# jonasrothfuss/ProMP

Measured on NVIDIA H100. Metric: env_steps_per_sec, higher is better.
Workload: dtype f32

## Files before the change

### promp_b200/csrc/policy_tc.cuh

```cuda
#pragma once
#include "mlp_tile.cuh"

namespace promp {

constexpr int TBT = 128;
constexpr int TC_HID = 64;
constexpr int SCA = TBT * 16 + 16;
constexpr int SCW = TC_HID * 16 + 16;
constexpr int TILE_A_BYTES = 16 * SCA;
constexpr int TILE_W_BYTES = 16 * SCW;

__device__ __forceinline__ int core_off(int r, int c, int sc) {
    return (c >> 2) * sc + (r >> 3) * 128 + (r & 7) * 16 + ((c & 3) << 2);
}
__device__ __forceinline__ float tf32_trunc(float x) { return __uint_as_float(__float_as_uint(x) & 0xffffe000u); }

template <int DO, int DA>
struct SmallLayout {
    static constexpr int W0 = 0;
    static constexpr int B0 = W0 + DO * TC_HID;
    static constexpr int B1 = B0 + TC_HID;
    static constexpr int W2 = B1 + TC_HID;
    static constexpr int B2 = W2 + TC_HID * DA;
    static constexpr int LS = B2 + DA;
    static constexpr int SIZE = (LS + DA + 3) / 4 * 4;
};

template <int DO, int DA, int NQ>
struct GradTcSmem {
    static constexpr int DOP = DOPad<DO>::V;
    alignas(16) unsigned char W1T_hi[TILE_W_BYTES];
    alignas(16) unsigned char W1T_lo[TILE_W_BYTES];
    alignas(16) unsigned char W1_hi[TILE_W_BYTES];
    alignas(16) unsigned char W1_lo[TILE_W_BYTES];
    alignas(16) unsigned char A0[TILE_A_BYTES];
    alignas(16) unsigned char A1[TILE_A_BYTES];
    alignas(16) unsigned char LO[TILE_A_BYTES];
    alignas(16) float Ps[SmallLayout<DO, DA>::SIZE];
    alignas(16) float X[TBT * DOP];
    float MUP[NQ * TBT * DA];
    float DMU[TBT * DA];
    float red[3 * 4 * NQ];
    HeadIn<DA> hin;
    HeadOld<DA> hold;
    int last;
};


__device__ __forceinline__ void mma_tf32_16n8k8(float (&c)[4], const uint32_t (&a)[4], const uint32_t (&b)[2]) {
    asm volatile("mma.sync.aligned.m16n8k8.row.col.f32.tf32.tf32.f32 {%0,%1,%2,%3}, {%4,%5,%6,%7}, {%8,%9}, {%0,%1,%2,%3};\n"
                 : "+f"(c[0]), "+f"(c[1]), "+f"(c[2]), "+f"(c[3])
                 : "r"(a[0]), "r"(a[1]), "r"(a[2]), "r"(a[3]), "r"(b[0]), "r"(b[1]));
}
__device__ __forceinline__ void split_tf32(float x, uint32_t& hi, uint32_t& lo) {
    hi = __float_as_uint(x) & 0xffffe000u;
    lo = __float_as_uint(x - __uint_as_float(hi));
}
template <bool COLSUM, int NT, bool UNIT = false>
__device__ __forceinline__ void wgrad_mma_tile(const unsigned char* __restrict__ At, const unsigned char* __restrict__ Dt,
                                               float scale, int warp, int lane, float (&acc)[NT][4], float (&csum)[NT]) {
    const int g = lane >> 2, t = lane & 3;
    const int k0 = 16 * (warp & 3) + g, j0 = 8 * NT * (warp >> 2) + g;
    const unsigned char* ap = At + (k0 >> 2) * SCA + (k0 & 3) * 4 + t * 32;
    const unsigned char* dp = Dt + (j0 >> 2) * SCA + (j0 & 3) * 4 + t * 32;
#pragma unroll 2
    for (int s = 0; s < TBT / 8; ++s) {
        uint32_t ah[4], al[4], bh[NT][2], bl[NT][2];
        split_tf32(*reinterpret_cast<const float*>(ap + s * 128), ah[0], al[0]);
        split_tf32(*reinterpret_cast<const float*>(ap + s * 128 + 2 * SCA), ah[1], al[1]);
        split_tf32(*reinterpret_cast<const float*>(ap + s * 128 + 16), ah[2], al[2]);
        split_tf32(*reinterpret_cast<const float*>(ap + s * 128 + 2 * SCA + 16), ah[3], al[3]);
#pragma unroll
        for (int nt = 0; nt < NT; ++nt) {
            const float d0 = *reinterpret_cast<const float*>(dp + nt * 2 * SCA + s * 128);
            const float d1 = *reinterpret_cast<const float*>(dp + nt * 2 * SCA + s * 128 + 16);
            if (COLSUM) csum[nt] += d0 + d1;
            split_tf32(UNIT ? d0 : scale * d0, bh[nt][0], bl[nt][0]);
            split_tf32(UNIT ? d1 : scale * d1, bh[nt][1], bl[nt][1]);
        }
#pragma unroll
        for (int nt = 0; nt < NT; ++nt) mma_tf32_16n8k8(acc[nt], al, bh[nt]);
#pragma unroll
        for (int nt = 0; nt < NT; ++nt) mma_tf32_16n8k8(acc[nt], ah, bl[nt]);
#pragma unroll
        for (int nt = 0; nt < NT; ++nt) mma_tf32_16n8k8(acc[nt], ah, bh[nt]);
    }
}
template <int NT>
__device__ __forceinline__ int wgrad_mma_index(int warp, int lane, int nt, int i) {
    const int g = lane >> 2, t = lane & 3;
    return (16 * (warp & 3) + g + 8 * (i >> 1)) * TC_HID + 8 * NT * (warp >> 2) + 8 * nt + 2 * t + (i & 1);
}

__device__ __forceinline__ uint64_t wg_desc(const unsigned char* p) {
    const uint32_t a = static_cast<uint32_t>(__cvta_generic_to_shared(p));
    return (uint64_t)((a & 0x3ffff) >> 4) | ((uint64_t)(SCW >> 4) << 16) | ((uint64_t)(128 >> 4) << 32);
}
__device__ __forceinline__ void wg_fence() { asm volatile("wgmma.fence.sync.aligned;\n" ::: "memory"); }
__device__ __forceinline__ void wg_commit() { asm volatile("wgmma.commit_group.sync.aligned;\n" ::: "memory"); }
__device__ __forceinline__ void wg_wait() { asm volatile("wgmma.wait_group.sync.aligned 0;\n" ::: "memory"); }
constexpr int WG_DEPTH = 0;
__device__ __forceinline__ void wg_wait_depth() { asm volatile("wgmma.wait_group.sync.aligned %0;\n" ::"n"(WG_DEPTH) : "memory"); }
__device__ __forceinline__ void wg_fence_weights() { asm volatile("fence.proxy.async.shared::cta;\n" ::: "memory"); }
template <int LNT>
__device__ __forceinline__ void wg_pin(float (&acc)[LNT][4]) {
#pragma unroll
    for (int nt = 0; nt < LNT; ++nt)
#pragma unroll
        for (int i = 0; i < 4; ++i) asm volatile("" : "+f"(acc[nt][i])::"memory");
}

template <int LNT>
__device__ __forceinline__ void wgmma_tf32(float (&d)[LNT][4], const uint32_t (&a)[4], uint64_t desc);
template <>
__device__ __forceinline__ void wgmma_tf32<4>(float (&d)[4][4], const uint32_t (&a)[4], uint64_t desc) {
    asm volatile(
        "wgmma.mma_async.sync.aligned.m64n32k8.f32.tf32.tf32 "
        "{%0,%1,%2,%3,%4,%5,%6,%7,%8,%9,%10,%11,%12,%13,%14,%15}, {%16,%17,%18,%19}, %20, 1, 1, 1;\n"
        : "+f"(d[0][0]), "+f"(d[0][1]), "+f"(d[0][2]), "+f"(d[0][3]), "+f"(d[1][0]), "+f"(d[1][1]), "+f"(d[1][2]), "+f"(d[1][3]),
          "+f"(d[2][0]), "+f"(d[2][1]), "+f"(d[2][2]), "+f"(d[2][3]), "+f"(d[3][0]), "+f"(d[3][1]), "+f"(d[3][2]), "+f"(d[3][3])
        : "r"(a[0]), "r"(a[1]), "r"(a[2]), "r"(a[3]), "l"(desc));
}
template <>
__device__ __forceinline__ void wgmma_tf32<8>(float (&d)[8][4], const uint32_t (&a)[4], uint64_t desc) {
    asm volatile(
        "wgmma.mma_async.sync.aligned.m64n64k8.f32.tf32.tf32 "
        "{%0,%1,%2,%3,%4,%5,%6,%7,%8,%9,%10,%11,%12,%13,%14,%15,"
        "%16,%17,%18,%19,%20,%21,%22,%23,%24,%25,%26,%27,%28,%29,%30,%31}, {%32,%33,%34,%35}, %36, 1, 1, 1;\n"
        : "+f"(d[0][0]), "+f"(d[0][1]), "+f"(d[0][2]), "+f"(d[0][3]), "+f"(d[1][0]), "+f"(d[1][1]), "+f"(d[1][2]), "+f"(d[1][3]),
          "+f"(d[2][0]), "+f"(d[2][1]), "+f"(d[2][2]), "+f"(d[2][3]), "+f"(d[3][0]), "+f"(d[3][1]), "+f"(d[3][2]), "+f"(d[3][3]),
          "+f"(d[4][0]), "+f"(d[4][1]), "+f"(d[4][2]), "+f"(d[4][3]), "+f"(d[5][0]), "+f"(d[5][1]), "+f"(d[5][2]), "+f"(d[5][3]),
          "+f"(d[6][0]), "+f"(d[6][1]), "+f"(d[6][2]), "+f"(d[6][3]), "+f"(d[7][0]), "+f"(d[7][1]), "+f"(d[7][2]), "+f"(d[7][3])
        : "r"(a[0]), "r"(a[1]), "r"(a[2]), "r"(a[3]), "l"(desc));
}
template <int LNT>
__device__ __forceinline__ void layer_gemm_issue(float (&acc)[LNT][4], const unsigned char* __restrict__ a,
                                                 const unsigned char* __restrict__ b_hi, const unsigned char* __restrict__ b_lo,
                                                 int warp, int lane) {
    const int g = lane >> 2, t = lane & 3;
    const unsigned char* ap = a + (warp & 7) * 256 + g * 16 + t * 4;
    const int bo = (warp >> 3) * LNT * 128;
#pragma unroll 1
    for (int s = 0; s < TC_HID / 8; ++s) {
        const uint64_t dh = wg_desc(b_hi + bo + 2 * s * SCW), dl = wg_desc(b_lo + bo + 2 * s * SCW);
        uint32_t ah[4], al[4];
        const unsigned char* as = ap + 2 * s * SCA;
        split_tf32(*reinterpret_cast<const float*>(as), ah[0], al[0]);
        split_tf32(*reinterpret_cast<const float*>(as + 128), ah[1], al[1]);
        split_tf32(*reinterpret_cast<const float*>(as + SCA), ah[2], al[2]);
        split_tf32(*reinterpret_cast<const float*>(as + SCA + 128), ah[3], al[3]);
        wg_fence();
        wgmma_tf32<LNT>(acc, al, dh);
        wgmma_tf32<LNT>(acc, ah, dl);
        wgmma_tf32<LNT>(acc, ah, dh);
        wg_commit();
        wg_wait_depth();
    }
}
template <int LNT>
__device__ __forceinline__ void zero_frag(float (&acc)[LNT][4]) {
#pragma unroll
    for (int nt = 0; nt < LNT; ++nt) acc[nt][0] = acc[nt][1] = acc[nt][2] = acc[nt][3] = 0.f;
}
template <int LNT>
__device__ __forceinline__ int frag_off(int warp, int lane, int nt, int h) {
    return core_off(16 * (warp & 7) + (lane >> 2) + 8 * h, 8 * (LNT * (warp >> 3) + nt) + 2 * (lane & 3), SCA);
}
template <int LNT>
__device__ __forceinline__ void store_frag(const float (&acc)[LNT][4], unsigned char* tile, int warp, int lane) {
#pragma unroll
    for (int nt = 0; nt < LNT; ++nt)
#pragma unroll
        for (int h = 0; h < 2; ++h)
            *reinterpret_cast<float2*>(tile + frag_off<LNT>(warp, lane, nt, h)) = make_float2(acc[nt][2 * h], acc[nt][2 * h + 1]);
}
template <int CW>
__device__ __forceinline__ void load_row(const unsigned char* tile, int r, int c0, float (&v)[CW]) {
#pragma unroll
    for (int c4 = 0; c4 < CW / 4; ++c4) {
        const float4 x = *reinterpret_cast<const float4*>(tile + core_off(r, c0 + 4 * c4, SCA));
        v[4 * c4] = x.x, v[4 * c4 + 1] = x.y, v[4 * c4 + 2] = x.z, v[4 * c4 + 3] = x.w;
    }
}

#ifdef PROMP_EXP_CLOCKS
__device__ unsigned long long g_chain_clk[16];
__device__ long long g_chain_last[1024];
#define CCLK(i)                                                                                  \
    do {                                                                                         \
        if (threadIdx.x == 0) {                                                                  \
            const long long t_ = clock64();                                                      \
            atomicAdd(&g_chain_clk[i], (unsigned long long)(t_ - g_chain_last[blockIdx.x]));     \
            g_chain_last[blockIdx.x] = t_;                                                       \
        }                                                                                        \
    } while (0)
#define CCNT(i)                                            \
    do {                                                   \
        if (threadIdx.x == 0) atomicAdd(&g_chain_clk[i], 1ull); \
    } while (0)
#else
#define CCLK(i)
#define CCNT(i)
#endif
struct ItemSched {
    int ntiles, g_lo, g_hi;
    int item, first_item, n_items;
    const int* ready_prev;
    int* ready_mine;
    __device__ __forceinline__ int my_slot(int) const { return item; }
    __device__ __forceinline__ int n_contrib(int) const { return n_items; }
    __device__ __forceinline__ int contrib_slot(int, int i) const { return first_item + i; }
    __device__ __forceinline__ void clk(int i) const { CCLK(i); }
    __device__ __forceinline__ void wait_task(int m) const {
        if (ready_prev == nullptr) return;
        if (threadIdx.x == 0) {
            int v;
            unsigned spins = 0;
            long long t0 = 0;
            do {
                asm volatile("ld.acquire.gpu.global.s32 %0, [%1];\n" : "=r"(v) : "l"(ready_prev + m) : "memory");
                if (v == 0 && (++spins & 0xfffu) == 0) {
                    const long long t = clock64();
                    if (t0 == 0) t0 = t;
                    else if (t - t0 > 8000000000ll) {
                        __trap();
                    }
                }
            } while (v == 0);
        }
        __syncthreads();
        CCLK(1);
    }
    __device__ __forceinline__ void publish_task(int m) const {
        __threadfence();
        __syncthreads();
        if (threadIdx.x == 0) asm volatile("st.release.gpu.global.s32 [%0], %1;\n" ::"l"(ready_mine + m), "r"(1) : "memory");
        CCNT(7);
    }
    static __device__ __forceinline__ float ldp(const float* p) { return __ldcg(p); }
    static __device__ __forceinline__ float4 ldp4(const float4* p) { return __ldcg(p); }
};

#ifdef PROMP_EXP_CLOCKS
__device__ unsigned long long g_phase_clk[16];
#define PCLK(i)                                                   \
    do {                                                          \
        if (blockIdx.x == 0 && threadIdx.x == 0) {                \
            const long long t_ = clock64();                       \
            s_clk[i] += (unsigned long long)(t_ - s_last);        \
            s_last = t_;                                          \
        }                                                         \
    } while (0)
#else
#define PCLK(i)
#endif
template <int DO, int DA, int NQ, class Act, class Sched, int ADV = ADV_SAMPLE>
__device__ __forceinline__ void grad_tc_tiles(const PolicyArgs& A, GradTcSmem<DO, DA, NQ>& S, const Sched& sc,
                                              const float*& cached_th) {
    constexpr int HID = TC_HID;
    using L = PLayout<DO, DA, HID>;
    using SL = SmallLayout<DO, DA>;
    using SM = GradTcSmem<DO, DA, NQ>;
    constexpr int TCT = 128 * NQ, CW = TC_HID / NQ, NW = TCT / 32, NT = 8 / NQ;
    constexpr int LNT = 64 / NW;
    constexpr int DOP = SM::DOP;
    constexpr int PSTRIDE = L::P + PSTAT;
    constexpr int NPART = TCT / HID, BPP = TBT / NPART;

#ifdef PROMP_EXP_CLOCKS
    __shared__ unsigned long long s_clk[16];
    __shared__ long long s_last;
    if (threadIdx.x == 0) {
        for (int i = 0; i < 16; ++i) s_clk[i] = 0;
        s_last = clock64();
    }
#endif

    const int tid = threadIdx.x, lane = tid & 31, warp = tid >> 5;
    const int qd = warp & 3, cq = warp >> 2;
    const int r = qd * 32 + lane, c0 = CW * cq;
    const int cj = tid & (HID - 1), cp = tid / HID;
    const int dO = obs_dim_of<DO, DA>(A), dA = act_dim_of<DO, DA>(A);
    const int N = A.N;
    const float kl_eff = kl_coeff_eff(A);
    float invN = 1.0f / (float)N;
    int Nm = N;
    const bool want_grad = A.grad != nullptr;
    const float* th = nullptr;
    HeadIn<DA>& hin = S.hin;

    float gW1[NT][4], gB1f[NT], gW0p[DO], gW2p[DA], gB0c, gB2w[DA], gLSw[DA];
    float s_obj, s_kl, s_ratio;
    auto zero_acc = [&]() {
#pragma unroll
        for (int a = 0; a < NT; ++a) gW1[a][0] = gW1[a][1] = gW1[a][2] = gW1[a][3] = gB1f[a] = 0.f;
#pragma unroll
        for (int i = 0; i < DO; ++i) gW0p[i] = 0.f;
#pragma unroll
        for (int d = 0; d < DA; ++d) gW2p[d] = 0.f;
#pragma unroll
        for (int d = 0; d < DA; ++d) gB2w[d] = gLSw[d] = 0.f;
        gB0c = 0.f;
        s_obj = s_kl = s_ratio = 0.f;
    };
    auto load_task = [&](int m) {
        sc.wait_task(m);
        if (A.n_valid) { Nm = __ldg(A.n_valid + m); invN = 1.0f / (float)max(Nm, 1); }
        th = A.params + (int64_t)m * A.param_stride;
        const bool reload = th != cached_th;
        cached_th = th;
        if (reload) __syncthreads();
        for (int i = tid; reload && i < DO * HID + HID; i += TCT) S.Ps[SL::W0 + i] = Sched::ldp(th + L::W0 + i);
        for (int i = tid; reload && i < HID; i += TCT) S.Ps[SL::B1 + i] = Sched::ldp(th + L::B1 + i);
        for (int i = tid; reload && i < HID * DA + 2 * DA; i += TCT) S.Ps[SL::W2 + i] = Sched::ldp(th + L::W2 + i);
        for (int u = tid; reload && u < HID * HID / 4; u += TCT) {
            float4 w, wl;
            {
                const int jg = u % (HID / 4), k = u / (HID / 4);
                w = Sched::ldp4(reinterpret_cast<const float4*>(th + L::W1 + k * HID + 4 * jg));
                wl = make_float4(w.x - tf32_trunc(w.x), w.y - tf32_trunc(w.y), w.z - tf32_trunc(w.z), w.w - tf32_trunc(w.w));
                const int off = jg * SCW + (k >> 3) * 128 + (k & 7) * 16;
                *reinterpret_cast<float4*>(S.W1_hi + off) = make_float4(tf32_trunc(w.x), tf32_trunc(w.y), tf32_trunc(w.z), tf32_trunc(w.w));
                *reinterpret_cast<float4*>(S.W1_lo + off) = wl;
            }
            {
                const int j = u % HID, kg = u / HID;
                const float* src = th + L::W1 + 4 * kg * HID + j;
// ... 154 lines not shown
                    mu[d] = sm;
                }
                float a[DA], mo[DA], lso[DA], adv;
                if constexpr (XPRE) {
#pragma unroll
                    for (int d = 0; d < DA; ++d) a[d] = ha[d], mo[d] = hmo[d], lso[d] = hlso[d];
                    adv = hadv;
                } else {
                    adv = load_head_sample<DA, ADV>(A, g0 + r, m, dA, A.ls_per_sample, a, mo, lso);
                }
                HeadOut<DA> o;
                out_forward<Act, DA>(mu);
                if (A.ls_per_sample) {
                    HeadOld<DA> ho;
                    head_old_from<DA>(lso, ho, dA);
                    gaussian_head<DA>(hin, ho, mu, a, mo, adv, A.obj_kind, A.clip_eps, o, dA);
                } else {
                    gaussian_head<DA>(hin, S.hold, mu, a, mo, adv, A.obj_kind, A.clip_eps, o, dA);
                }
                grad_signal<DA>(hin, o, A.obj_scale, kl_eff, invN, dmu, dls);
                out_grad_back<Act, DA>(mu, dmu);
                s_obj += o.obj;
                s_kl += o.kl;
                s_ratio += o.ratio;
            } else {
#pragma unroll
                for (int d = 0; d < DA; ++d) dmu[d] = dls[d] = 0.f;
            }
#pragma unroll
            for (int d = 0; d < DA; ++d) {
                S.DMU[r * DA + d] = dmu[d];
                gB2w[d] += dmu[d], gLSw[d] += dls[d];
            }
        }
        if (!want_grad) continue;
        __syncthreads();
        PCLK(4);
        {
            const int b0 = cp * BPP;
            const unsigned char* colp = S.A1 + core_off(b0, cj, SCA);
            const float* dmu0 = S.DMU + b0 * DA;
#pragma unroll(BPP <= 16 ? 2 : 1)
            for (int b8 = 0; b8 < BPP; b8 += 8)
#pragma unroll
            for (int b1 = 0; b1 < 8; ++b1) {
                const int bb = b8 + b1;
                const float h = *reinterpret_cast<const float*>(colp + (bb >> 3) * 128 + (bb & 7) * 16);
#pragma unroll
                for (int d = 0; d < DA; ++d) gW2p[d] = fmaf(h, dmu0[bb * DA + d], gW2p[d]);
            }
        }
        __syncthreads();
        PCLK(5);
        {
            float dm[DA];
#pragma unroll
            for (int d = 0; d < DA; ++d) dm[d] = S.DMU[r * DA + d];
#pragma unroll
            for (int c4 = 0; c4 < CW / 4; ++c4) {
                float v[4];
#pragma unroll
                for (int e = 0; e < 4; ++e) {
                    const int c = 4 * c4 + e;
                    float dh = 0.f;
#pragma unroll
                    for (int d = 0; d < DA; ++d) dh = fmaf(dm[d], S.Ps[SL::W2 + (c0 + c) * DA + d], dh);
                    v[e] = dh * Act::d(h2[c]);
                }
                *reinterpret_cast<float4*>(S.A1 + core_off(r, c0 + 4 * c4, SCA)) = make_float4(v[0], v[1], v[2], v[3]);
            }
        }
        __syncthreads();
        PCLK(6);
        wgrad_mma_tile<true, NT, true>(S.A0, S.A1, 1.f, warp, lane, gW1, gB1f);
        PCLK(7);
        {
            float acc[LNT][4];
            zero_frag<LNT>(acc);
            layer_gemm_issue<LNT>(acc, S.A1, S.W1_hi, S.W1_lo, warp, lane);
            wg_wait();
            wg_pin<LNT>(acc);
            __syncthreads();
            PCLK(8);
#pragma unroll
            for (int nt = 0; nt < LNT; ++nt)
#pragma unroll
                for (int h = 0; h < 2; ++h) {
                    float2* p = reinterpret_cast<float2*>(S.A0 + frag_off<LNT>(warp, lane, nt, h));
                    const float2 hv = *p;
                    *p = make_float2(acc[nt][2 * h] * Act::d(hv.x), acc[nt][2 * h + 1] * Act::d(hv.y));
                }
        }
        __syncthreads();
        PCLK(9);
        {
            const int b0 = cp * BPP;
            const unsigned char* colp = S.A0 + core_off(b0, cj, SCA);
            const float* x0 = S.X + b0 * DOP;
#pragma unroll(BPP <= 16 ? 2 : 1)
            for (int b8 = 0; b8 < BPP; b8 += 8)
#pragma unroll
            for (int b1 = 0; b1 < 8; ++b1) {
                const int bb = b8 + b1;
                const float d1 = *reinterpret_cast<const float*>(colp + (bb >> 3) * 128 + (bb & 7) * 16);
                gB0c += d1;
#pragma unroll
                for (int i = 0; i < DO; ++i) gW0p[i] = fmaf(x0[bb * DOP + i], d1, gW0p[i]);
            }
        }
    }
    PCLK(10);
    if (cur_m >= 0) flush(cur_m);
    PCLK(11);
#ifdef PROMP_EXP_CLOCKS
    if (blockIdx.x == 0 && threadIdx.x == 0)
        for (int i = 0; i < 16; ++i) g_phase_clk[i] += s_clk[i];
#endif
}

template <int DO, int DA, int NQ, class Act, int ADV = ADV_SAMPLE>
__device__ __forceinline__ void policy_grad_tc_body(const PolicyArgs& A) {
    using SM = GradTcSmem<DO, DA, NQ>;
    using L = PLayout<DO, DA, TC_HID>;
    extern __shared__ __align__(16) unsigned char smem_raw[];
    SM& S = *reinterpret_cast<SM*>(smem_raw);
    if (reuse_hit<L::P>(A.skip_flag, A.params, A.skip_theta)) return;
    reuse_produce<L::P, L::LS, DA>(A);
    const UniformSched sc(A.M, A.N, A.q, A.kmax, TBT);
    const float* cached_th = nullptr;
    grad_tc_tiles<DO, DA, NQ, Act, UniformSched, ADV>(A, S, sc, cached_th);
}
template <int DO, int DA, int NQ>
__global__ void __launch_bounds__(128 * NQ, 1) policy_grad_tc_kernel(PolicyArgs A) { policy_grad_tc_body<DO, DA, NQ, ActTanh>(A); }
template <int DO, int DA, int NQ>
__global__ void __launch_bounds__(128 * NQ, 1) policy_grad_tc_relu_kernel(PolicyArgs A) { policy_grad_tc_body<DO, DA, NQ, ActRelu>(A); }
template <int DO, int DA, int NQ>
__global__ void __launch_bounds__(128 * NQ, 1) policy_grad_tc_explore_kernel(PolicyArgs A) {
    policy_grad_tc_body<DO, DA, NQ, ActTanh, ADV_TASK>(A);
}
template <int DO, int DA, int NQ>
__global__ void __launch_bounds__(128 * NQ, 1) policy_grad_tc_explore_relu_kernel(PolicyArgs A) {
    policy_grad_tc_body<DO, DA, NQ, ActRelu, ADV_TASK>(A);
}
template <int DO, int DA, int NQ, class Hid>
__global__ void __launch_bounds__(128 * NQ, 1) policy_grad_tc_otanh_kernel(PolicyArgs A) {
    policy_grad_tc_body<DO, DA, NQ, OutTanh<Hid>>(A);
}
template <int DO, int DA, int NQ, class Hid>
__global__ void __launch_bounds__(128 * NQ, 1) policy_grad_tc_explore_otanh_kernel(PolicyArgs A) {
    policy_grad_tc_body<DO, DA, NQ, OutTanh<Hid>, ADV_TASK>(A);
}


template <int DO, int DA, int NQ>
struct HvpTcSmem {
    static constexpr int DOP = DOPad<DO>::V;
    alignas(16) unsigned char WB[4][TILE_W_BYTES];
    alignas(16) unsigned char H1[TILE_A_BYTES];
    alignas(16) unsigned char R1[TILE_A_BYTES];
    alignas(16) unsigned char T2a[TILE_A_BYTES];
    alignas(16) unsigned char T2b[TILE_A_BYTES];
    alignas(16) float Ps[SmallLayout<DO, DA>::SIZE];
    alignas(16) float Vs[SmallLayout<DO, DA>::SIZE];
    float DMU[TBT * DA];
    float CMU[TBT * DA];
    float red[3 * 4 * NQ];
    HeadIn<DA> hin;
    HeadOld<DA> hold;
    int last;
};

template <int DO, int DA, int NQ, class Act, class Sched>
__device__ __forceinline__ void hvp_tc_tiles(const PolicyArgs& A, HvpTcSmem<DO, DA, NQ>& S, const Sched& sc,
                                             const float*& cached_th) {
    constexpr int HID = TC_HID;
    using L = PLayout<DO, DA, HID>;
    using SL = SmallLayout<DO, DA>;
    using SM = HvpTcSmem<DO, DA, NQ>;
    constexpr int TCT = 128 * NQ, CW = TC_HID / NQ, NW = TCT / 32, NT = 8 / NQ;
    constexpr int LNT = 64 / NW;
    constexpr int DOP = SM::DOP;
    constexpr int PSTRIDE = L::P + PSTAT;
    constexpr int NPART = TCT / HID, BPP = TBT / NPART;

    float* const sX = reinterpret_cast<float*>(S.T2a);
    float* const sMUP = reinterpret_cast<float*>(S.WB[0]);
    static_assert(TBT * DOP * 4 <= TILE_A_BYTES && NQ * TBT * 2 * DA * 4 <= 2 * TILE_W_BYTES, "aliased buffers must fit");

    const int tid = threadIdx.x, lane = tid & 31, warp = tid >> 5;
    const int qd = warp & 3, cq = warp >> 2;
    const int r = qd * 32 + lane, c0 = CW * cq;
    const int cj = tid & (HID - 1), cp = tid / HID;
    const int dO = obs_dim_of<DO, DA>(A), dA = act_dim_of<DO, DA>(A);
    const int N = A.N;
    const float kl_eff = kl_coeff_eff(A);
    float invN = 1.0f / (float)N;
    int Nm = N;
    const float ac = -A.inner_lr;
    const float* th = nullptr;
    const float* vg = nullptr;
    HeadIn<DA>& hin = S.hin;
    float rls[DA];

    float gW1[NT][4], gB1f[NT], gW0p[DO], gW2p[DA], gB0c, gB2w[DA], gLSw[DA];
    float s_obj, s_kl, s_ratio;
    auto zero_acc = [&]() {
#pragma unroll
        for (int a = 0; a < NT; ++a) gW1[a][0] = gW1[a][1] = gW1[a][2] = gW1[a][3] = gB1f[a] = 0.f;
#pragma unroll
        for (int i = 0; i < DO; ++i) gW0p[i] = 0.f;
#pragma unroll
        for (int d = 0; d < DA; ++d) gW2p[d] = 0.f;
#pragma unroll
        for (int d = 0; d < DA; ++d) gB2w[d] = gLSw[d] = 0.f;
        gB0c = 0.f;
        s_obj = s_kl = s_ratio = 0.f;
    };
    const bool vec_ro = A.out != A.vec;
    const float* const al = A.step_size;
    auto ldv = [&](const float* p) {
        const float v = vec_ro ? Sched::ldp(p) : __ldcg(p);
        return al ? __ldg(al + (p - vg)) * v : v;
    };
    auto ldv4 = [&](const float4* p) {
        const float4 v = vec_ro ? Sched::ldp4(p) : __ldcg(p);
        if (!al) return v;
        const float4 a = __ldg(reinterpret_cast<const float4*>(al + (reinterpret_cast<const float*>(p) - vg)));
        return make_float4(a.x * v.x, a.y * v.y, a.z * v.z, a.w * v.w);
    };
    auto load_task = [&](int m) {
        sc.wait_task(m);
        if (A.n_valid) { Nm = __ldg(A.n_valid + m); invN = 1.0f / (float)max(Nm, 1); }
        th = A.params + (int64_t)m * A.param_stride;
        vg = A.vec + (int64_t)m * L::P;
        __syncthreads();
        const bool reload_p = th != cached_th;
        cached_th = th;
        for (int i = tid; i < DO * HID + HID; i += TCT) {
            if (reload_p) S.Ps[SL::W0 + i] = Sched::ldp(th + L::W0 + i);
            S.Vs[SL::W0 + i] = ldv(vg + L::W0 + i);
        }
        for (int i = tid; i < HID; i += TCT) {
            if (reload_p) S.Ps[SL::B1 + i] = Sched::ldp(th + L::B1 + i);
            S.Vs[SL::B1 + i] = ldv(vg + L::B1 + i);
        }
        for (int i = tid; i < HID * DA + 2 * DA; i += TCT) {
            if (reload_p) S.Ps[SL::W2 + i] = Sched::ldp(th + L::W2 + i);
            S.Vs[SL::W2 + i] = ldv(vg + L::W2 + i);
        }
        __syncthreads();
        if (tid == 0) head_setup<DA>(A, S.Ps + SL::LS, m, dA, hin, &S.hold);
        __syncthreads();
#pragma unroll
        for (int d = 0; d < DA; ++d) rls[d] = S.Vs[SL::LS + d] * hin.ls_mask[d];
    };
    auto load_weights = [&](bool fwd) {
        for (int u = tid; u < HID * HID / 4; u += TCT) {
            float4 w, v;
            int off;
            if (fwd) {
                const int j = u % HID, kg = u / HID;
                const float* sw = th + L::W1 + 4 * kg * HID + j;
                const float* sv = vg + L::W1 + 4 * kg * HID + j;
                w = make_float4(Sched::ldp(sw), Sched::ldp(sw + HID), Sched::ldp(sw + 2 * HID), Sched::ldp(sw + 3 * HID));
                v = make_float4(ldv(sv), ldv(sv + HID), ldv(sv + 2 * HID), ldv(sv + 3 * HID));
                off = kg * SCW + (j >> 3) * 128 + (j & 7) * 16;
            } else {
                const int jg = u % (HID / 4), k = u / (HID / 4);
                w = Sched::ldp4(reinterpret_cast<const float4*>(th + L::W1 + k * HID + 4 * jg));
                v = ldv4(reinterpret_cast<const float4*>(vg + L::W1 + k * HID + 4 * jg));
                v = make_float4(ac * v.x, ac * v.y, ac * v.z, ac * v.w);
                off = jg * SCW + (k >> 3) * 128 + (k & 7) * 16;
            }
            *reinterpret_cast<float4*>(S.WB[0] + off) = make_float4(tf32_trunc(w.x), tf32_trunc(w.y), tf32_trunc(w.z), tf32_trunc(w.w));
            *reinterpret_cast<float4*>(S.WB[1] + off) =
                make_float4(w.x - tf32_trunc(w.x), w.y - tf32_trunc(w.y), w.z - tf32_trunc(w.z), w.w - tf32_trunc(w.w));
            *reinterpret_cast<float4*>(S.WB[2] + off) = make_float4(tf32_trunc(v.x), tf32_trunc(v.y), tf32_trunc(v.z), tf32_trunc(v.w));
            *reinterpret_cast<float4*>(S.WB[3] + off) =
                make_float4(v.x - tf32_trunc(v.x), v.y - tf32_trunc(v.y), v.z - tf32_trunc(v.z), v.w - tf32_trunc(v.w));
        }
        wg_fence_weights();
    };
    auto flush = [&](int m) {
        sc.clk(3);
        float* part = A.partial + (int64_t)sc.my_slot(m) * PSTRIDE;
        float* scr = reinterpret_cast<float*>(S.T2a);
        __syncthreads();
#pragma unroll
        for (int nt = 0; nt < NT; ++nt)
#pragma unroll
            for (int i = 0; i < 4; ++i) part[L::W1 + wgrad_mma_index<NT>(warp, lane, nt, i)] = gW1[nt][i];
#pragma unroll
        for (int nt = 0; nt < NT; ++nt) {
            float c = gB1f[nt];
            c += __shfl_xor_sync(0xffffffffu, c, 1);
            c += __shfl_xor_sync(0xffffffffu, c, 2);
            if ((lane & 3) == 0 && (warp & 3) == 0) part[L::B1 + 8 * NT * (warp >> 2) + 8 * nt + (lane >> 2)] = c;
        }
        scr[cp * HID + cj] = gB0c;
        __syncthreads();
        if (tid < HID) {
            float s = 0.f;
            for (int p = 0; p < NPART; ++p) s += scr[p * HID + tid];
            part[L::B0 + tid] = s;
        }
        __syncthreads();
#pragma unroll
        for (int d = 0; d < DA; ++d) {
            const float s1 = warp_sum(gB2w[d]), s2 = warp_sum(gLSw[d]);
            if (cq == 0 && lane == 0) scr[qd * 2 * DA + d] = s1, scr[qd * 2 * DA + DA + d] = s2;
        }
        __syncthreads();
        if (tid < 2 * DA) part[L::B2 + tid] = scr[tid] + scr[2 * DA + tid] + scr[4 * DA + tid] + scr[6 * DA + tid];
        __syncthreads();
        flush_tail<TCT, 8, 2 * TILE_A_BYTES / 4, DO, DA, HID>(A, sc, m, invN, true, part, scr, S.red, S.last, gW0p, gW2p, s_obj, s_kl, s_ratio,
                                        HvpEpilogue<L::P>{A, vg, m});
    };

    constexpr int XR = (TBT * DOP) / TCT;
    constexpr bool XPRE = (TBT * DOP) % TCT == 0 && XR >= 1 && XR <= 2 && DA <= 2;
    float xq[XPRE ? XR : 1], xc[XPRE ? XR : 1], ha[DA], hmo[DA], hlso[DA], hadv = 0.f;
    auto fetch_x = [&](int g_, float (&dst)[XPRE ? XR : 1]) {
        const int m_ = g_ / sc.ntiles, n0_ = (g_ - m_ * sc.ntiles) * TBT;
        const int nb_ = max(0, min(TBT, (A.n_valid ? __ldg(A.n_valid + m_) : N) - n0_));
#pragma unroll
        for (int e = 0; e < (XPRE ? XR : 1); ++e) {
            const int i = tid + e * TCT, b = i / DOP, c = i % DOP;
            dst[e] = (b < nb_ && c < dO) ? __ldg(A.obs + ((int64_t)m_ * N + n0_ + b) * dO + c) : 0.f;
        }
    };
    int cur_m = -1;
    for (int g = sc.g_lo; g < sc.g_hi; ++g) {
        const int m = g / sc.ntiles, tile = g - m * sc.ntiles;
        if (m != cur_m) {
            if (cur_m >= 0) flush(cur_m);
            load_task(m);
            sc.clk(2);
            zero_acc();
            cur_m = m;
        }
        const int n0 = tile * TBT, nb = max(0, min(TBT, Nm - n0));
        const int64_t g0 = (int64_t)m * N + n0;
        __syncthreads();
        auto load_x = [&]() {
            for (int i = tid; i < TBT * DOP; i += TCT) {
                const int b = i / DOP, c = i % DOP;
                sX[i] = (b < nb && c < dO) ? __ldg(A.obs + (g0 + b) * dO + c) : 0.f;
            }
        };
        if constexpr (XPRE) {
            if (g == sc.g_lo) fetch_x(g, xq);
#pragma unroll
            for (int e = 0; e < XR; ++e) xc[e] = xq[e], sX[tid + e * TCT] = xc[e];
            if (g + 1 < sc.g_hi) fetch_x(g + 1, xq);
            if (cq == 0 && r < nb) hadv = load_head_sample<DA>(A, g0 + r, m, dA, A.ls_per_sample, ha, hmo, hlso);
        } else {
            load_x();
        }
        load_weights(true);
        __syncthreads();
        {
            float x[DO];
#pragma unroll
            for (int i = 0; i < DO; ++i) x[i] = sX[r * DOP + i];
#pragma unroll
            for (int c4 = 0; c4 < CW / 4; ++c4) {
                float h[4], r1[4];
#pragma unroll
                for (int e = 0; e < 4; ++e) {
                    const int c = c0 + 4 * c4 + e;
                    float z = S.Ps[SL::B0 + c], rz = S.Vs[SL::B0 + c];
#pragma unroll
                    for (int i = 0; i < DO; ++i) {
                        z = fmaf(x[i], S.Ps[SL::W0 + i * HID + c], z);
                        rz = fmaf(x[i], S.Vs[SL::W0 + i * HID + c], rz);
                    }
                    h[e] = Act::f(z);
                    r1[e] = Act::d(h[e]) * rz;
                }
                const int off = core_off(r, c0 + 4 * c4, SCA);
                *reinterpret_cast<float4*>(S.H1 + off) = make_float4(h[0], h[1], h[2], h[3]);
                *reinterpret_cast<float4*>(S.R1 + off) = make_float4(r1[0], r1[1], r1[2], r1[3]);
            }
        }
        __syncthreads();
        {
            float acc[LNT][4];
            zero_frag<LNT>(acc);
            layer_gemm_issue<LNT>(acc, S.H1, S.WB[0], S.WB[1], warp, lane);
            wg_wait();
            wg_pin<LNT>(acc);
            store_frag<LNT>(acc, S.T2a, warp, lane);
            zero_frag<LNT>(acc);
            layer_gemm_issue<LNT>(acc, S.R1, S.WB[0], S.WB[1], warp, lane);
            layer_gemm_issue<LNT>(acc, S.H1, S.WB[2], S.WB[3], warp, lane);
            wg_wait();
            wg_pin<LNT>(acc);
            store_frag<LNT>(acc, S.T2b, warp, lane);
        }
        __syncthreads();
        float h2[CW], r2[CW];
        load_row<CW>(S.T2a, r, c0, h2);
        load_row<CW>(S.T2b, r, c0, r2);
        {
            float mup[DA], rmup[DA];
#pragma unroll
            for (int d = 0; d < DA; ++d) mup[d] = rmup[d] = 0.f;
#pragma unroll
            for (int c4 = 0; c4 < CW / 4; ++c4) {
#pragma unroll
                for (int e = 0; e < 4; ++e) {
                    const int c = 4 * c4 + e;
                    h2[c] = Act::f(h2[c] + S.Ps[SL::B1 + c0 + c]);
                    r2[c] = Act::d(h2[c]) * (r2[c] + S.Vs[SL::B1 + c0 + c]);
#pragma unroll
                    for (int d = 0; d < DA; ++d) {
                        const float w2 = S.Ps[SL::W2 + (c0 + c) * DA + d];
                        mup[d] = fmaf(h2[c], w2, mup[d]);
                        rmup[d] = fmaf(r2[c], w2, fmaf(h2[c], S.Vs[SL::W2 + (c0 + c) * DA + d], rmup[d]));
                    }
                }
                const int off = core_off(r, c0 + 4 * c4, SCA);
                *reinterpret_cast<float4*>(S.T2a + off) = make_float4(h2[4 * c4], h2[4 * c4 + 1], h2[4 * c4 + 2], h2[4 * c4 + 3]);
                *reinterpret_cast<float4*>(S.T2b + off) = make_float4(r2[4 * c4], r2[4 * c4 + 1], r2[4 * c4 + 2], r2[4 * c4 + 3]);
            }
#pragma unroll
            for (int d = 0; d < DA; ++d) {
                sMUP[((cq * TBT + r) * 2 + 0) * DA + d] = mup[d];
                sMUP[((cq * TBT + r) * 2 + 1) * DA + d] = rmup[d];
            }
        }
        __syncthreads();
        if (cq == 0) {
            float dmu[DA], cmu[DA], cls[DA];
            if (r < nb) {
                float mu[DA], rmu[DA];
#pragma unroll
                for (int d = 0; d < DA; ++d) {
                    float sm = S.Ps[SL::B2 + d], sr = S.Vs[SL::B2 + d];
#pragma unroll
                    for (int q = 0; q < NQ; ++q) sm += sMUP[((q * TBT + r) * 2 + 0) * DA + d], sr += sMUP[((q * TBT + r) * 2 + 1) * DA + d];
                    mu[d] = sm;
                    rmu[d] = sr;
                }
                float a[DA], mo[DA], lso[DA], adv;
                if constexpr (XPRE) {
#pragma unroll
                    for (int d = 0; d < DA; ++d) a[d] = ha[d], mo[d] = hmo[d], lso[d] = hlso[d];
                    adv = hadv;
                } else {
                    adv = load_head_sample<DA>(A, g0 + r, m, dA, A.ls_per_sample, a, mo, lso);
                }
                HeadOut<DA> o;
                out_forward_tangent<Act, DA>(mu, rmu);
                if (A.ls_per_sample) {
                    HeadOld<DA> ho;
                    head_old_from<DA>(lso, ho, dA);
                    gaussian_head<DA>(hin, ho, mu, a, mo, adv, A.obj_kind, A.clip_eps, o, dA);
                } else {
                    gaussian_head<DA>(hin, S.hold, mu, a, mo, adv, A.obj_kind, A.clip_eps, o, dA);
                }
                hvp_signal<DA>(hin, o, rmu, rls, A.obj_kind, kl_eff, invN, ac, dA, dmu, cmu, cls);
                out_hvp_back<Act, DA>(mu, rmu, ac, dmu, cmu);
                s_obj += o.obj;
                s_kl += o.kl;
                s_ratio += o.ratio;
            } else {
#pragma unroll
                for (int d = 0; d < DA; ++d) dmu[d] = cmu[d] = cls[d] = 0.f;
            }
#pragma unroll
            for (int d = 0; d < DA; ++d) {
                S.DMU[r * DA + d] = dmu[d], S.CMU[r * DA + d] = cmu[d];
                gB2w[d] += cmu[d], gLSw[d] += cls[d];
            }
        }
        __syncthreads();
        load_weights(false);
        {
            const int b0 = cp * BPP;
            const int off0 = core_off(b0, cj, SCA);
            const float* cmu0 = S.CMU + b0 * DA;
            const float* dmu0 = S.DMU + b0 * DA;
#pragma unroll(BPP <= 16 ? 2 : 1)
            for (int b8 = 0; b8 < BPP; b8 += 8)
#pragma unroll
            for (int b1 = 0; b1 < 8; ++b1) {
                const int bb = b8 + b1;
                const int off = off0 + (bb >> 3) * 128 + (bb & 7) * 16;
                const float h = *reinterpret_cast<const float*>(S.T2a + off);
                const float rr = ac * *reinterpret_cast<const float*>(S.T2b + off);
#pragma unroll
                for (int d = 0; d < DA; ++d) gW2p[d] = fmaf(h, cmu0[bb * DA + d], fmaf(rr, dmu0[bb * DA + d], gW2p[d]));
            }
        }
        __syncthreads();
        {
            float dm[DA], cm[DA];
#pragma unroll
            for (int d = 0; d < DA; ++d) dm[d] = S.DMU[r * DA + d], cm[d] = S.CMU[r * DA + d];
#pragma unroll
            for (int c4 = 0; c4 < CW / 4; ++c4) {
                float d2[4], c2[4];
#pragma unroll
                for (int e = 0; e < 4; ++e) {
                    const int c = 4 * c4 + e;
                    float dh = 0.f, ch = 0.f;
#pragma unroll
                    for (int d = 0; d < DA; ++d) {
                        const float w2 = S.Ps[SL::W2 + (c0 + c) * DA + d], v2 = S.Vs[SL::W2 + (c0 + c) * DA + d];
                        dh = fmaf(dm[d], w2, dh);
                        ch = fmaf(cm[d], w2, fmaf(ac * dm[d], v2, ch));
                    }
                    d2[e] = dh * Act::d(h2[c]);
                    c2[e] = act_hvp_back<Act>(ch, dh, h2[c], r2[c], ac);
                }
                const int off = core_off(r, c0 + 4 * c4, SCA);
                *reinterpret_cast<float4*>(S.T2a + off) = make_float4(d2[0], d2[1], d2[2], d2[3]);
                *reinterpret_cast<float4*>(S.T2b + off) = make_float4(c2[0], c2[1], c2[2], c2[3]);
            }
        }
        __syncthreads();
        {
            float unused[NT] = {};
            wgrad_mma_tile<true, NT, true>(S.H1, S.T2b, 1.f, warp, lane, gW1, gB1f);
            wgrad_mma_tile<false, NT>(S.R1, S.T2a, ac, warp, lane, gW1, unused);
        }
        {
            float dacc[LNT][4], cacc[LNT][4];
            zero_frag<LNT>(dacc);
            zero_frag<LNT>(cacc);
            layer_gemm_issue<LNT>(dacc, S.T2a, S.WB[0], S.WB[1], warp, lane);
            layer_gemm_issue<LNT>(cacc, S.T2b, S.WB[0], S.WB[1], warp, lane);
            layer_gemm_issue<LNT>(cacc, S.T2a, S.WB[2], S.WB[3], warp, lane);
            wg_wait();
            wg_pin<LNT>(dacc);
            wg_pin<LNT>(cacc);
            __syncthreads();
#pragma unroll
            for (int nt = 0; nt < LNT; ++nt)
#pragma unroll
                for (int h = 0; h < 2; ++h) {
                    const int off = frag_off<LNT>(warp, lane, nt, h);
                    float2* p = reinterpret_cast<float2*>(S.H1 + off);
                    const float2 hv = *p;
                    const float2 rv = *reinterpret_cast<const float2*>(S.R1 + off);
                    const float dx = dacc[nt][2 * h], dy = dacc[nt][2 * h + 1];
                    *p = make_float2(act_hvp_back<Act>(cacc[nt][2 * h], dx, hv.x, rv.x, ac),
                                     act_hvp_back<Act>(cacc[nt][2 * h + 1], dy, hv.y, rv.y, ac));
                }
        }
        if constexpr (XPRE) {
#pragma unroll
            for (int e = 0; e < XR; ++e) sX[tid + e * TCT] = xc[e];
        } else {
            load_x();
        }
        __syncthreads();
        {
            const int b0 = cp * BPP;
            const unsigned char* colp = S.H1 + core_off(b0, cj, SCA);
            const float* x0 = sX + b0 * DOP;
#pragma unroll(BPP <= 16 ? 2 : 1)
            for (int b8 = 0; b8 < BPP; b8 += 8)
#pragma unroll
            for (int b1 = 0; b1 < 8; ++b1) {
                const int bb = b8 + b1;
                const float c1 = *reinterpret_cast<const float*>(colp + (bb >> 3) * 128 + (bb & 7) * 16);
                gB0c += c1;
#pragma unroll
                for (int i = 0; i < DO; ++i) gW0p[i] = fmaf(x0[bb * DOP + i], c1, gW0p[i]);
            }
        }
    }
    if (cur_m >= 0) flush(cur_m);
}

template <int DO, int DA, int NQ, class Act>
__device__ __forceinline__ void policy_hvp_tc_body(const PolicyArgs& A) {
    using SM = HvpTcSmem<DO, DA, NQ>;
    extern __shared__ __align__(16) unsigned char smem_raw[];
    SM& S = *reinterpret_cast<SM*>(smem_raw);
    const UniformSched sc(A.M, A.N, A.q, A.kmax, TBT);
    const float* cached_th = nullptr;
    hvp_tc_tiles<DO, DA, NQ, Act>(A, S, sc, cached_th);
}
template <int DO, int DA, int NQ>
__global__ void __launch_bounds__(128 * NQ, 1) policy_hvp_tc_kernel(PolicyArgs A) { policy_hvp_tc_body<DO, DA, NQ, ActTanh>(A); }
template <int DO, int DA, int NQ>
__global__ void __launch_bounds__(128 * NQ, 1) policy_hvp_tc_relu_kernel(PolicyArgs A) { policy_hvp_tc_body<DO, DA, NQ, ActRelu>(A); }
template <int DO, int DA, int NQ, class Hid>
__global__ void __launch_bounds__(128 * NQ, 1) policy_hvp_tc_otanh_kernel(PolicyArgs A) {
    policy_hvp_tc_body<DO, DA, NQ, OutTanh<Hid>>(A);
}

constexpr int CHAIN_MAX_STAGES = 6;
constexpr int CHAIN_MAX_REGIONS = 3;
struct ChainStageInfo {
    int kind;
    int ntiles;
    int item_base, n_items;
    int n_regions;
    int reg_m0[CHAIN_MAX_REGIONS + 1];
    int reg_q[CHAIN_MAX_REGIONS];
    int reg_item0[CHAIN_MAX_REGIONS];
};
struct ChainArgs {
    int n_stages, n_items, M;
    int* ctrl;
    int* ready;
    const int* skip_flag;
    const float* skip_theta;
    ChainStageInfo info[CHAIN_MAX_STAGES];
    PolicyArgs st[CHAIN_MAX_STAGES];
};

template <int DO, int DA, int NQ>
struct ChainSmem {
    static constexpr int BODY = (int)((sizeof(GradTcSmem<DO, DA, NQ>) > sizeof(HvpTcSmem<DO, DA, NQ>) ? sizeof(GradTcSmem<DO, DA, NQ>)
                                                                                                    : sizeof(HvpTcSmem<DO, DA, NQ>)) + 15) / 16 * 16;
    static constexpr int SIZE = BODY + 16;
};

#if defined(PROMP_POLICY_RELU_TU) && defined(PROMP_POLICY_OTANH_TU)
#define PROMP_CHAIN_KERNEL policy_chain_tc_relu_otanh_kernel
using ChainAct = OutTanh<ActRelu>;
#elif defined(PROMP_POLICY_OTANH_TU)
#define PROMP_CHAIN_KERNEL policy_chain_tc_otanh_kernel
using ChainAct = OutTanh<ActTanh>;
#elif defined(PROMP_POLICY_RELU_TU)
#define PROMP_CHAIN_KERNEL policy_chain_tc_relu_kernel
using ChainAct = ActRelu;
#else
#define PROMP_CHAIN_KERNEL policy_chain_tc_kernel
using ChainAct = ActTanh;
#endif
template <int DO, int DA, int NQ, bool HAS_HVP = true, int ADV = ADV_SAMPLE>
__global__ void __launch_bounds__(128 * NQ, 1) PROMP_CHAIN_KERNEL(const __grid_constant__ ChainArgs C) {
    using Act = ChainAct;
    using GS = GradTcSmem<DO, DA, NQ>;
    using HS = HvpTcSmem<DO, DA, NQ>;
    using L = PLayout<DO, DA, TC_HID>;
    extern __shared__ __align__(16) unsigned char smem_raw[];
    GS& G = *reinterpret_cast<GS*>(smem_raw);
    HS& H = *reinterpret_cast<HS*>(smem_raw);
    int* cur_item = reinterpret_cast<int*>(smem_raw + ChainSmem<DO, DA, NQ>::BODY);
    const int tid = threadIdx.x;

    const bool skip0 = reuse_hit<L::P>(C.skip_flag, C.st[0].params, C.skip_theta);
#ifdef PROMP_EXP_CLOCKS
    if (tid == 0) g_chain_last[blockIdx.x] = clock64();
    const long long t_begin = clock64();
#endif
    const float* cached_g = nullptr;
    const float* cached_h = nullptr;
    for (;;) {
        __syncthreads();
        if (tid == 0) *cur_item = atomicAdd(C.ctrl, 1);
        __syncthreads();
        const int it = *cur_item;
        if (it >= C.n_items) break;
        CCNT(6);
        int s = 0;
        while (s + 1 < C.n_stages && it >= C.info[s + 1].item_base) ++s;
        if (s == 0 && skip0) continue;
        const ChainStageInfo& I = C.info[s];
        const int j = it - I.item_base;
        int r = 0;
        while (r + 1 < I.n_regions && j >= I.reg_item0[r + 1]) ++r;
        const int q = I.reg_q[r], per_task = (I.ntiles + q - 1) / q;
        const int jr = j - I.reg_item0[r];
        const int mr = jr / per_task, k = jr - mr * per_task;
        const int m = I.reg_m0[r] + mr;
        ItemSched sc;
        sc.ntiles = I.ntiles;
        sc.g_lo = m * I.ntiles + k * q;
        sc.g_hi = m * I.ntiles + min(k * q + q, I.ntiles);
        sc.item = it;
        sc.first_item = I.item_base + I.reg_item0[r] + mr * per_task;
        sc.n_items = per_task;
        sc.ready_prev = (s > 0 && !(s == 1 && skip0)) ? C.ready + (s - 1) * C.M : nullptr;
        if constexpr (ADV == ADV_EITHER)
            if (C.st[s].adv_per_task) sc.ready_prev = nullptr;
        sc.ready_mine = C.ready + s * C.M;
        CCLK(0);
        if (!HAS_HVP || I.kind == 0) {
            cached_h = nullptr;
            grad_tc_tiles<DO, DA, NQ, Act, ItemSched, ADV>(C.st[s], G, sc, cached_g);
        } else if constexpr (HAS_HVP) {
            cached_g = nullptr;
            hvp_tc_tiles<DO, DA, NQ, Act>(C.st[s], H, sc, cached_h);
        }
    }
#ifdef PROMP_EXP_CLOCKS
    if (tid == 0) {
        atomicAdd(&g_chain_clk[8], (unsigned long long)(clock64() - t_begin));
        atomicAdd(&g_chain_clk[9], 1ull);
    }
#endif
    if (tid == 0) {
        __threadfence();
        if (atomicAdd(C.ctrl + 1, 1) == (int)gridDim.x - 1) {
            for (int i = 0; i < C.n_stages * C.M; ++i) C.ready[i] = 0;
            C.ctrl[0] = 0;
            C.ctrl[1] = 0;
            __threadfence();
        }
    }
}

}
```

Measured before the change: 100.0 million.

## Keep HVP weight tiles resident in shared memory and transpose forward GEMM

When shared memory allows, the HVP kernel now loads W1 and the scaled V1 hi/lo TF32 splits once per task into extra resident weight buffers, instead of reloading weights every tile. It also adds a transposed forward wgmma path that uses weights as the register A operand and activations as shared-memory descriptors. This path precomputes activation low parts to fuse the R-forward pass. The aim is to cut per-tile global weight loads and conversion work, at the cost of more shared memory and a separate X/MU buffer. Clock probes are added under an experimental macro.

```diff
diff --git a/promp_b200/csrc/policy_tc.cuh b/promp_b200/csrc/policy_tc.cuh
--- a/promp_b200/csrc/policy_tc.cuh
+++ b/promp_b200/csrc/policy_tc.cuh
@@ -92,9 +92,9 @@
     return (16 * (warp & 3) + g + 8 * (i >> 1)) * TC_HID + 8 * NT * (warp >> 2) + 8 * nt + 2 * t + (i & 1);
 }
 
-__device__ __forceinline__ uint64_t wg_desc(const unsigned char* p) {
+__device__ __forceinline__ uint64_t wg_desc(const unsigned char* p, int lbo = SCW) {
     const uint32_t a = static_cast<uint32_t>(__cvta_generic_to_shared(p));
-    return (uint64_t)((a & 0x3ffff) >> 4) | ((uint64_t)(SCW >> 4) << 16) | ((uint64_t)(128 >> 4) << 32);
+    return (uint64_t)((a & 0x3ffff) >> 4) | ((uint64_t)(lbo >> 4) << 16) | ((uint64_t)(128 >> 4) << 32);
 }
 __device__ __forceinline__ void wg_fence() { asm volatile("wgmma.fence.sync.aligned;\n" ::: "memory"); }
 __device__ __forceinline__ void wg_commit() { asm volatile("wgmma.commit_group.sync.aligned;\n" ::: "memory"); }
@@ -173,6 +173,70 @@
 #pragma unroll
         for (int h = 0; h < 2; ++h)
             *reinterpret_cast<float2*>(tile + frag_off<LNT>(warp, lane, nt, h)) = make_float2(acc[nt][2 * h], acc[nt][2 * h + 1]);
+}
+__device__ __forceinline__ int fwd_unit(int warp, int i) {
+    const int p = 2 * (warp & 3) + (i >> 3), g = i & 7;
+    return 4 * ((p & 3) + 8 * (p >> 2) + 4 * (g >> 2)) + (g & 3);
+}
+template <int LNT>
+__device__ __forceinline__ void fwd_gemm_t_issue(float (&z)[LNT][4], float (&rz)[LNT][4], const unsigned char* __restrict__ h1,
+                                                 const unsigned char* __restrict__ h1lo, const unsigned char* __restrict__ r1,
+                                                 const unsigned char* __restrict__ r1lo, const unsigned char* __restrict__ w_hi,
+                                                 const unsigned char* __restrict__ w_lo, const unsigned char* __restrict__ v,
+                                                 int warp, int lane) {
+    const int g = lane >> 2, t = lane & 3;
+    const int j0 = fwd_unit(warp, g), j1 = fwd_unit(warp, g + 8);
+    const int o0 = (j0 >> 2) * SCW + (j0 & 3) * 4 + t * 16, o1 = (j1 >> 2) * SCW + (j1 & 3) * 4 + t * 16;
+    const int bo = (warp >> 2) * LNT * 128;
+    auto frag = [&](const unsigned char* w, int s, uint32_t (&a)[4]) {
+        a[0] = *reinterpret_cast<const uint32_t*>(w + o0 + s * 128);
+        a[1] = *reinterpret_cast<const uint32_t*>(w + o1 + s * 128);
+        a[2] = *reinterpret_cast<const uint32_t*>(w + o0 + s * 128 + 64);
+        a[3] = *reinterpret_cast<const uint32_t*>(w + o1 + s * 128 + 64);
+    };
+#pragma unroll 1
+    for (int s = 0; s < TC_HID / 8; ++s) {
+        const uint64_t dh = wg_desc(h1 + bo + 2 * s * SCA, SCA), dhl = wg_desc(h1lo + bo + 2 * s * SCA, SCA);
+        const uint64_t dr = wg_desc(r1 + bo + 2 * s * SCA, SCA), drl = wg_desc(r1lo + bo + 2 * s * SCA, SCA);
+        uint32_t wh[4], wl[4];
+        frag(w_hi, s, wh);
+        frag(w_lo, s, wl);
+        wg_fence();
+        wgmma_tf32<LNT>(z, wh, dhl);
+        wgmma_tf32<LNT>(z, wl, dh);
+        wgmma_tf32<LNT>(z, wh, dh);
+        wgmma_tf32<LNT>(rz, wh, drl);
+        wgmma_tf32<LNT>(rz, wl, dr);
+        wgmma_tf32<LNT>(rz, wh, dr);
+        wg_commit();
+        wg_wait_depth();
+    }
+#pragma unroll 1
+    for (int s = 0; s < TC_HID / 8; ++s) {
+        const uint64_t dh = wg_desc(h1 + bo + 2 * s * SCA, SCA), dhl = wg_desc(h1lo + bo + 2 * s * SCA, SCA);
+        uint32_t raw[4], vh[4], vl[4];
+        frag(v, s, raw);
+#pragma unroll
+        for (int i = 0; i < 4; ++i) split_tf32(__uint_as_float(raw[i]), vh[i], vl[i]);
+        wg_fence();
+        wgmma_tf32<LNT>(rz, vh, dhl);
+        wgmma_tf32<LNT>(rz, vl, dh);
+        wgmma_tf32<LNT>(rz, vh, dh);
+        wg_commit();
+        wg_wait_depth();
+    }
+}
+template <int LNT>
+__device__ __forceinline__ void store_frag_t(const float (&acc)[LNT][4], unsigned char* tile, int warp, int lane) {
+    const int b0 = (warp >> 2) * LNT * 8 + 2 * (lane & 3);
+#pragma unroll
+    for (int h = 0; h < 2; ++h) {
+        const int j = fwd_unit(warp, (lane >> 2) + 8 * h);
+#pragma unroll
+        for (int nt = 0; nt < LNT; ++nt)
+#pragma unroll
+            for (int e = 0; e < 2; ++e) *reinterpret_cast<float*>(tile + core_off(b0 + 8 * nt + e, j, SCA)) = acc[nt][2 * h + e];
+    }
 }
 template <int CW>
 __device__ __forceinline__ void load_row(const unsigned char* tile, int r, int c0, float (&v)[CW]) {
@@ -633,10 +697,12 @@
 }
 
 
-template <int DO, int DA, int NQ>
-struct HvpTcSmem {
+template <int DO, int DA, int NQ, bool RES_>
+struct HvpTcSmemT {
     static constexpr int DOP = DOPad<DO>::V;
-    alignas(16) unsigned char WB[4][TILE_W_BYTES];
+    static constexpr bool RES = RES_;
+    static constexpr int XM_FLOATS = RES ? (TBT * DOP > NQ * TBT * 2 * DA ? TBT * DOP : NQ * TBT * 2 * DA) : 4;
+    alignas(16) unsigned char WB[RES ? 5 : 4][TILE_W_BYTES];
     alignas(16) unsigned char H1[TILE_A_BYTES];
     alignas(16) unsigned char R1[TILE_A_BYTES];
     alignas(16) unsigned char T2a[TILE_A_BYTES];
@@ -649,7 +715,12 @@
     HeadIn<DA> hin;
     HeadOld<DA> hold;
     int last;
+    alignas(16) float XM[XM_FLOATS];
 };
+template <int DO, int DA, int NQ>
+constexpr bool hvp_resident() { return sizeof(HvpTcSmemT<DO, DA, NQ, true>) + 16 <= 227 * 1024; }
+template <int DO, int DA, int NQ>
+using HvpTcSmem = HvpTcSmemT<DO, DA, NQ, hvp_resident<DO, DA, NQ>()>;
 
 template <int DO, int DA, int NQ, class Act, class Sched>
 __device__ __forceinline__ void hvp_tc_tiles(const PolicyArgs& A, HvpTcSmem<DO, DA, NQ>& S, const Sched& sc,
@@ -663,10 +734,20 @@
     constexpr int DOP = SM::DOP;
     constexpr int PSTRIDE = L::P + PSTAT;
     constexpr int NPART = TCT / HID, BPP = TBT / NPART;
-
-    float* const sX = reinterpret_cast<float*>(S.T2a);
-    float* const sMUP = reinterpret_cast<float*>(S.WB[0]);
+    constexpr bool RES = SM::RES;
+
+    float* const sX = RES ? S.XM : reinterpret_cast<float*>(S.T2a);
+    float* const sMUP = RES ? S.XM : reinterpret_cast<float*>(S.WB[0]);
     static_assert(TBT * DOP * 4 <= TILE_A_BYTES && NQ * TBT * 2 * DA * 4 <= 2 * TILE_W_BYTES, "aliased buffers must fit");
+
+#ifdef PROMP_EXP_CLOCKS
+    __shared__ unsigned long long s_clk[16];
+    __shared__ long long s_last;
+    if (threadIdx.x == 0) {
+        for (int i = 0; i < 16; ++i) s_clk[i] = 0;
+        s_last = clock64();
+    }
+#endif
 
     const int tid = threadIdx.x, lane = tid & 31, warp = tid >> 5;
     const int qd = warp & 3, cq = warp >> 2;
@@ -729,6 +810,25 @@
             if (reload_p) S.Ps[SL::W2 + i] = Sched::ldp(th + L::W2 + i);
             S.Vs[SL::W2 + i] = ldv(vg + L::W2 + i);
         }
+        if constexpr (RES) {
+            for (int u = tid; u < HID * HID / 4; u += TCT) {
+                const int jg = u % (HID / 4), k = u / (HID / 4);
+                const int off = jg * SCW + (k >> 3) * 128 + (k & 7) * 16;
+                if (reload_p) {
+                    const float4 w = Sched::ldp4(reinterpret_cast<const float4*>(th + L::W1 + k * HID + 4 * jg));
+                    *reinterpret_cast<float4*>(S.WB[0] + off) = make_float4(tf32_trunc(w.x), tf32_trunc(w.y), tf32_trunc(w.z), tf32_trunc(w.w));
+                    *reinterpret_cast<float4*>(S.WB[1] + off) =
+                        make_float4(w.x - tf32_trunc(w.x), w.y - tf32_trunc(w.y), w.z - tf32_trunc(w.z), w.w - tf32_trunc(w.w));
+                }
+                float4 v = ldv4(reinterpret_cast<const float4*>(vg + L::W1 + k * HID + 4 * jg));
+                *reinterpret_cast<float4*>(S.WB[4] + off) = v;
+                v = make_float4(ac * v.x, ac * v.y, ac * v.z, ac * v.w);
+                *reinterpret_cast<float4*>(S.WB[2] + off) = make_float4(tf32_trunc(v.x), tf32_trunc(v.y), tf32_trunc(v.z), tf32_trunc(v.w));
+                *reinterpret_cast<float4*>(S.WB[3] + off) =
+                    make_float4(v.x - tf32_trunc(v.x), v.y - tf32_trunc(v.y), v.z - tf32_trunc(v.z), v.w - tf32_trunc(v.w));
+            }
+            wg_fence_weights();
+        }
         __syncthreads();
         if (tid == 0) head_setup<DA>(A, S.Ps + SL::LS, m, dA, hin, &S.hold);
         __syncthreads();
@@ -813,12 +913,15 @@
     int cur_m = -1;
     for (int g = sc.g_lo; g < sc.g_hi; ++g) {
         const int m = g / sc.ntiles, tile = g - m * sc.ntiles;
+        PCLK(10);
         if (m != cur_m) {
             if (cur_m >= 0) flush(cur_m);
+            PCLK(11);
             load_task(m);
             sc.clk(2);
             zero_acc();
             cur_m = m;
+            PCLK(12);
         }
         const int n0 = tile * TBT, nb = max(0, min(TBT, Nm - n0));
         const int64_t g0 = (int64_t)m * N + n0;
@@ -838,8 +941,10 @@
         } else {
             load_x();
         }
-        load_weights(true);
-        __syncthreads();
+        PCLK(0);
+        if constexpr (!RES) load_weights(true);
+        __syncthreads();
+        PCLK(1);
         {
             float x[DO];
 #pragma unroll
@@ -862,10 +967,29 @@
                 const int off = core_off(r, c0 + 4 * c4, SCA);
                 *reinterpret_cast<float4*>(S.H1 + off) = make_float4(h[0], h[1], h[2], h[3]);
                 *reinterpret_cast<float4*>(S.R1 + off) = make_float4(r1[0], r1[1], r1[2], r1[3]);
-            }
-        }
-        __syncthreads();
-        {
+                if constexpr (RES) {
+                    *reinterpret_cast<float4*>(S.T2a + off) =
+                        make_float4(h[0] - tf32_trunc(h[0]), h[1] - tf32_trunc(h[1]), h[2] - tf32_trunc(h[2]), h[3] - tf32_trunc(h[3]));
+                    *reinterpret_cast<float4*>(S.T2b + off) =
+                        make_float4(r1[0] - tf32_trunc(r1[0]), r1[1] - tf32_trunc(r1[1]), r1[2] - tf32_trunc(r1[2]), r1[3] - tf32_trunc(r1[3]));
+                }
+            }
+        }
+        if constexpr (RES) wg_fence_weights();
+        __syncthreads();
+        PCLK(2);
+        if constexpr (RES) {
+            float z[LNT][4], rz[LNT][4];
+            zero_frag<LNT>(z);
+            zero_frag<LNT>(rz);
+            fwd_gemm_t_issue<LNT>(z, rz, S.H1, S.T2a, S.R1, S.T2b, S.WB[0], S.WB[1], S.WB[4], warp, lane);
+            wg_wait();
+            wg_pin<LNT>(z);
+            wg_pin<LNT>(rz);
+            __syncthreads();
+            store_frag_t<LNT>(z, S.T2a, warp, lane);
+            store_frag_t<LNT>(rz, S.T2b, warp, lane);
+        } else {
             float acc[LNT][4];
             zero_frag<LNT>(acc);
             layer_gemm_issue<LNT>(acc, S.H1, S.WB[0], S.WB[1], warp, lane);
@@ -880,6 +1004,7 @@
             store_frag<LNT>(acc, S.T2b, warp, lane);
         }
         __syncthreads();
+        PCLK(3);
         float h2[CW], r2[CW];
         load_row<CW>(S.T2a, r, c0, h2);
         load_row<CW>(S.T2b, r, c0, r2);
@@ -912,6 +1037,7 @@
             }
         }
         __syncthreads();
+        PCLK(4);
         if (cq == 0) {
             float dmu[DA], cmu[DA], cls[DA];
             if (r < nb) {
@@ -957,7 +1083,9 @@
             }
         }
         __syncthreads();
-        load_weights(false);
+        PCLK(5);
+        if constexpr (!RES) load_weights(false);
+        PCLK(6);
         {
             const int b0 = cp * BPP;
             const int off0 = core_off(b0, cj, SCA);
@@ -976,6 +1104,7 @@
             }
         }
         __syncthreads();
+        PCLK(7);
         {
             float dm[DA], cm[DA];
 #pragma unroll
@@ -1002,11 +1131,13 @@
             }
         }
         __syncthreads();
+        PCLK(8);
         {
             float unused[NT] = {};
             wgrad_mma_tile<true, NT, true>(S.H1, S.T2b, 1.f, warp, lane, gW1, gB1f);
             wgrad_mma_tile<false, NT>(S.R1, S.T2a, ac, warp, lane, gW1, unused);
         }
+        PCLK(9);
         {
             float dacc[LNT][4], cacc[LNT][4];
             zero_frag<LNT>(dacc);
@@ -1031,6 +1162,7 @@
                                      act_hvp_back<Act>(cacc[nt][2 * h + 1], dy, hv.y, rv.y, ac));
                 }
         }
+        PCLK(13);
         if constexpr (XPRE) {
 #pragma unroll
             for (int e = 0; e < XR; ++e) sX[tid + e * TCT] = xc[e];
@@ -1038,6 +1170,7 @@
             load_x();
         }
         __syncthreads();
+        PCLK(14);
         {
             const int b0 = cp * BPP;
             const unsigned char* colp = S.H1 + core_off(b0, cj, SCA);
@@ -1054,7 +1187,13 @@
             }
         }
     }
+    PCLK(10);
     if (cur_m >= 0) flush(cur_m);
+    PCLK(11);
+#ifdef PROMP_EXP_CLOCKS
+    if (blockIdx.x == 0 && threadIdx.x == 0)
+        for (int i = 0; i < 16; ++i) g_phase_clk[i] += s_clk[i];
+#endif
 }
 
 template <int DO, int DA, int NQ, class Act>
```

New measurement: 102.0 million, median of 6. 1.02x the previous value.
